# borodark/exmc

Measured on AMD Instinct MI355X. Metric: leapfrog_steps_per_s, higher is better.
Workload: dtype f64; 1 GPU; eight_schools d=10, 4096 chains/GPU (4096 total), 138450 draws/chain (2769 steps of 50 draws) after one shared 1000-iteration warmup, max_tree_depth 10, target_accept 0.8; draws_per_chain=138450, lanes_per_chain=16, warmup_lanes_per_chain=16, seed=42

## Files before the change

exmc_amd/csrc/exmc_device.hpp:

```cpp
#pragma once

#include <hip/hip_runtime.h>
#include <stdint.h>
#include <type_traits>

#include <utility>

#include "../../include/exmc_detmath.h"

namespace exmc {

constexpr uint64_t kMask58 = (1ULL << 58) - 1;

#ifndef EXMC_FIXED_PART_PIECES
#define EXMC_FIXED_PART_PIECES 7
#endif

__device__ __forceinline__ bool div_in_range(double x) {
  const uint32_t h = (uint32_t)__double2hiint(x) & 0x7fffffffu;
  return (h - 0x28300000u) < (0x57C00000u - 0x28300000u);
}

struct Recip {
  double b, r;
};

__device__ __forceinline__ Recip make_recip(double b) { return Recip{b, exmc_rcp_refined(b)}; }

__device__ __forceinline__ Recip make_recip_literal(double b) {
  __asm__ volatile("" : "+v"(b));
  return make_recip(b);
}

template <bool kFast>
struct Div {
  bool ok = true;
  __device__ __forceinline__ void watch(double x) {
    if (kFast) ok = ok && div_in_range(x);
  }
  __device__ __forceinline__ void watch_if(bool relevant, double x) {
    if (kFast) ok = ok && (!relevant || div_in_range(x));
  }
  template <int ELO, int EHI>
  __device__ __forceinline__ void watch_exp_if(bool relevant, double x) {
    static_assert(ELO >= -380 && EHI <= 380 && ELO < EHI, "inside the division window");
    if (kFast) {
      const uint32_t h = (uint32_t)__double2hiint(x) & 0x7fffffffu;
      const bool in = (h - ((uint32_t)(1023 + ELO) << 20)) < ((uint32_t)(EHI - ELO) << 20);
      ok = ok && (!relevant || in);
    }
  }
  __device__ __forceinline__ double operator()(double a, const Recip& c) const {
    return kFast ? exmc_div_core(a, c.b, c.r) : (a / c.b);
  }
  __device__ __forceinline__ double operator()(double a, double b) const {
    return kFast ? exmc_div_core(a, b, exmc_rcp_refined(b)) : (a / b);
  }
};

template <class F>
__device__ __forceinline__ double with_fast_div(F&& f) {
  Div<true> fast;
  double r = f(fast);
  if (__builtin_expect(__any(fast.ok ? 0 : 1) != 0, 0)) {
    Div<false> exact;
    r = f(exact);
  }
  return r;
// ... 1087 lines not shown
```

exmc_amd/csrc/exmc_models.hpp:

```cpp
#pragma once

#include "exmc_device.hpp"

namespace exmc {

__device__ __forceinline__ double clamp200(double z) { return fmax(-200.0, fmin(z, 200.0)); }

struct ModelDefaults {
  static constexpr bool kVregMath = false;
  static constexpr bool kCoop = false;
  static constexpr int kExtraLdsDoubles = 0;
  static constexpr int kStageDoubles = 0;
  template <class C>
  __host__ static bool stage_ok(const C&) { return true; }
  static constexpr int kStageRowOffset = 0;
  static constexpr int kLdsDataDoubles = 0;
  static constexpr bool kPipeWarmup = true;
  static constexpr bool kHasPipeWarmup = true;
  static constexpr bool kXRowLds = false;
  static constexpr bool kRowDense = false;
  static constexpr bool kLaneDense = false;
  static constexpr bool kDenseImage = false;
  static constexpr int kDenseLdsDoubles = 0;
  static constexpr int kNutsWavesPerSimd = 1;
  static constexpr bool kRngOrbit = false;
  static constexpr bool kMigrate = false;
  static constexpr double kPrioRateWith = 1.0, kPrioRateWithout = 1.0;
  static constexpr int kPipeNutsLevels = 0;
  static constexpr bool kNutsZigInLds = true;
  static constexpr bool kRegradProposal = false;
  static constexpr int kWgWaves = 0;
  static constexpr int kWgLdsLevels = 1;
  static constexpr int kWgImageDoubles = 0;
  template <class C>
  __host__ __device__ static bool wg_ok(const C&) { return false; }
  static constexpr bool kLeafPairs = false;
  static constexpr bool kLeafPairExp = false;
  static constexpr bool kLeanMomentum = false;
  static constexpr bool kPassExpPairs = false;
  static constexpr bool kOuterLogPair = false;
  static constexpr bool kTreePrefix = false;
  static constexpr bool kRngWindow = false;
  static constexpr bool kPackedTrace = false;
};

extern __shared__ double exmc_dyn_lds[];
typedef double exmc_v2d __attribute__((ext_vector_type(2)));
typedef __attribute__((address_space(3))) exmc_v2d lds_v2d;
typedef __attribute__((address_space(3))) double lds_f64_m;
static __device__ const double exmc_logtab_dev[2 * EXMC_LOGTAB_ENTRIES] = {EXMC_LOGTAB_VALUES};
__device__ static __forceinline__ double exmc_log_tab_global(double x) {
  double m;
  int e;
  const int i = exmc_logtab_split(x, &m, &e);
  return exmc_logtab_finish(m, e, exmc_logtab_dev[2 * i], exmc_logtab_dev[2 * i + 1]);
}

struct EightSchoolsConsts {
  double y[8], sg[8], lsg[8];
  double c_mu;
  double c_hc;
  double c1;
};

template <int G>
struct EightSchools : ModelDefaults {
  static constexpr int D = 10;
  static constexpr int DPL = (D + G - 1) / G;
  static constexpr bool kVregMath = (DPL <= 2);
#ifndef EXMC_ES_PIPE_LEVELS
#define EXMC_ES_PIPE_LEVELS 2
#endif
  static constexpr int kPipeNutsLevels = (G == 16) ? EXMC_ES_PIPE_LEVELS : 0;
  static constexpr bool kLeafPairs = (G == 16);
  static constexpr bool kLeafPairExp = (G == 16);
  static constexpr bool kLeanMomentum = (G == 16);
  static constexpr bool kOuterLogPair = (G == 16);
  static constexpr bool kTreePrefix = (G == 16);
  static constexpr bool kRngWindow = (G == 16);
  static constexpr bool kPackedTrace = (G == 16);
  using MM = Math<kVregMath>;
  using Consts = EightSchoolsConsts;
  struct Lane {
    double y[DPL], lsg[DPL];
    Recip sg[DPL];
    Recip five;
    double cc;
  };

  __device__ static __forceinline__ void load(const Consts& c, int l, Lane& ln) {
#pragma unroll
    for (int k = 0; k < DPL; k++) {
      const int i = l + k * G;
      const int j = (i >= 2 && i < D) ? (i - 2) : 0;
      ln.y[k] = c.y[j];
      ln.sg[k] = make_recip(c.sg[j]);
      ln.lsg[k] = c.lsg[j];
    }
    ln.five = make_recip_literal(5.0);
    ln.cc = (l == 0) ? c.c_mu : c.c1;
  }

  __device__ static __forceinline__ double logp_grad(const Consts& c, const Lane& ln, int l,
                                                     const double (&q)[DPL], double (&g)[DPL]) {
    return with_fast_div([&](auto& dv) -> double { return eval(c, ln, l, q, g, dv); });
  }

  template <class DV>
  __device__ static __forceinline__ double eval(const Consts& c, const Lane& ln, int l,
                                                const double (&q)[DPL], double (&g)[DPL], DV& dv) {
    if constexpr (kSeqSum<G, D>) return eval_row(c, ln, l, q, g, dv);
    else return eval_slots(c, ln, l, q, g, dv);
  }

  struct Mid {
    double den, zc, T, lik;
  };
  template <class DV>
  __device__ static __forceinline__ void eval_row_grad(const Consts& c, const Lane& ln, int l,
                                                       const double (&q)[DPL], double (&g)[DPL], DV& dv,
                                                       Mid& m) {
    static_assert(DPL == 1, "one dimension per lane");
    const double mu = group_bcast_c<G, 0>(q[0]);
    const double zraw = group_bcast_c<G, 1>(q[0]);
    const double zc = clamp200(zraw);
    const double tau = MM::exp_pm200(zc);
    const bool isth = (l >= 2) && (l < D);
    const bool l0 = (l == 0), l1 = (l == 1);
    const double th = q[0];
    const double theta = mu + tau * th;
    const double resid = ln.y[0] - theta;
    constexpr bool kThetaLanes = (EXMC_ROW_SUM_PIECES & 1) != 0, kOneWatch = (EXMC_ROW_SUM_PIECES & 4) != 0;
// ... 1173 lines not shown
      g[k] = (-ar) + sj * sa;
    }
    if constexpr (G == 64) rs64_allsum6(s);
    else group_allsum_n<G, 6>(s);
    const bool in_a = (zsa_raw > -200.0) && (zsa_raw < 200.0);
    const bool in_y = (zsy_raw > -200.0) && (zsy_raw < 200.0);
    if constexpr (kSpread) {
      constexpr int ks = J / G;
      const int j = l + ks * G;
      const bool is_mu = j == J, is_g = j == J + 1, is_a = j == J + 2, is_y = j == J + 3, is_b = j == J + 4;
      const double v = is_mu ? mu : (is_g ? gam : beta);
      Recip rc;
      rc.b = is_mu ? ln.ten.b : ln.five.b;
      rc.r = is_mu ? ln.ten.r : ln.five.r;
      const double cst = is_mu ? ln.kc[kMu10] : ln.kc[kN5];
      const double sx = is_mu ? s[1] : (is_g ? s[2] : s[4]);
      const double zn = dv(v - 0.0, rc);
      const double Tn = -0.5 * (zn * zn + cst);
      const double gn = (-dv(zn, rc)) + sx;
      const double zc = is_a ? za : zy, zc2 = is_a ? za2 : zy2;
      const double dc = -dv(dv(2.0 * zc, ln.c25), 1.0 + zc2);
      const double ga = in_a ? ((dc + s[3]) * sa + 1.0) : 0.0;
      const double gy = in_y ? ((dc * sy + s[5]) + 1.0) : 0.0;
      const bool is_n = is_mu || is_g || is_b;
      T[ks] = is_n ? Tn : (is_a ? t_sa : (is_y ? t_sy : T[ks]));
      g[ks] = is_n ? gn : (is_a ? ga : (is_y ? gy : g[ks]));
#pragma unroll
      for (int k = 0; k < DPL; k++)
        if (l + k * G >= D) g[k] = 0.0;
      return group_sum_slots<G, DPL>(T, valid, l, s[0]);
    }
    const double zmu = dv(mu - 0.0, ln.ten), zg = dv(gam - 0.0, ln.five), zb = dv(beta - 0.0, ln.five);
#pragma unroll
    for (int k = 0; k < DPL; k++) {
      const int j = l + k * G;
      if (j == J) { T[k] = -0.5 * (zmu * zmu + ln.kc[kMu10]); g[k] = (-dv(zmu, ln.ten)) + s[1]; }
      if (j == J + 1) { T[k] = -0.5 * (zg * zg + ln.kc[kN5]); g[k] = (-dv(zg, ln.five)) + s[2]; }
      if (j == J + 2) { T[k] = t_sa; g[k] = in_a ? ((dsa + s[3]) * sa + 1.0) : 0.0; }
      if (j == J + 3) { T[k] = t_sy; g[k] = in_y ? ((dsy * sy + s[5]) + 1.0) : 0.0; }
      if (j == J + 4) { T[k] = -0.5 * (zb * zb + ln.kc[kN5]); g[k] = (-dv(zb, ln.five)) + s[4]; }
      if (j >= D) g[k] = 0.0;
    }
    return group_sum_slots<G, DPL>(T, valid, l, s[0]);
  }
};

template <class M>
struct RowDenseModel : M {
  static constexpr bool kRowDense = true;
  static constexpr bool kPipeWarmup = false;
  static constexpr bool kOuterLogPair = false;
  static constexpr bool kTreePrefix = false;
  static constexpr bool kRngWindow = false;
  static constexpr bool kPackedTrace = false;
  static_assert(M::DPL == 1 && M::D <= 12, "row layout: one dimension per lane, D <= 12");
};

template <class M, int G>
struct LaneDenseModel : M {
  static constexpr bool kLaneDense = true;
  static constexpr bool kPipeWarmup = false;
  static constexpr int kNutsWavesPerSimd = 1;
  static constexpr int kPipeNutsLevels = 0;
  static constexpr bool kDenseImage = M::D * M::D * 8 <= 16 * 1024;
  static constexpr int kDenseLdsDoubles = (64 / G) * 3 * M::D + (kDenseImage ? M::D * M::D + 64 : 0);
  static_assert(G >= 16 && M::DPL * G >= M::D && !M::kCoop, "a lane layout that holds the whole chain");
};

}

#ifdef EXMC_CUSTOM_HEADER
#define EXMC_GEN_HOST static inline
#define EXMC_GEN_FN static __host__ __device__ __forceinline__
static __host__ __device__ __noinline__ double exmc_gen_exp_call(double x) { return exmc_exp(x); }
static __host__ __device__ __noinline__ double exmc_gen_log_call(double x) { return exmc_log(x); }
static __host__ __device__ __noinline__ double exmc_gen_log1p_call(double x) { return exmc_log1p(x); }
static __host__ __device__ __noinline__ double exmc_gen_erf_call(double x) { return exmc_erf(x); }
#define EXMC_GEN_ERF exmc_gen_erf_call
#define EXMC_GENV_ERF exmc_gen_erf_call
#ifdef EXMC_GEN_INLINE_MATH
#define EXMC_GEN_EXP exmc_exp
#define EXMC_GEN_LOG exmc_log
#define EXMC_GEN_LOG1P exmc_log1p
#else
#define EXMC_GEN_EXP exmc_gen_exp_call
#define EXMC_GEN_LOG exmc_gen_log_call
#define EXMC_GEN_LOG1P exmc_gen_log1p_call
#endif
#ifdef EXMC_GENV_CALLED_MATH
#define EXMC_GENV_EXP exmc_gen_exp_call
#define EXMC_GENV_LOG exmc_gen_log_call
#define EXMC_GENV_LOG1P exmc_gen_log1p_call
#else
#define EXMC_GENV_EXP exmc_exp
#define EXMC_GENV_LOG exmc_log
#define EXMC_GENV_LOG1P exmc_log1p
#endif
#ifdef EXMC_GENL_CALLED_MATH
#define EXMC_GENL_EXP exmc_gen_exp_call
#define EXMC_GENL_LOG exmc_gen_log_call
#define EXMC_GENL_LOG1P exmc_gen_log1p_call
#else
#define EXMC_GENL_EXP exmc::Math<true>::exp
#define EXMC_GENL_LOG exmc::Math<true>::log
#define EXMC_GENL_LOG1P exmc_log1p
#endif
// ... 409 lines not shown
```

exmc_amd/csrc/exmc_nuts.hpp:

```cpp
#pragma once

#include <type_traits>

#include "exmc_models.hpp"

#ifndef EXMC_ABLATE
#define EXMC_ABLATE 0
#endif

#ifndef EXMC_PROFILE_SECTIONS
#define EXMC_PROFILE_SECTIONS 0
#endif

namespace exmc {

#ifdef EXMC_XCC_PROBE
__device__ double g_wave_probe[4096 * 5];
#endif

#if EXMC_PROFILE_SECTIONS
__device__ unsigned long long g_prof[16];
#define EXMC_PROF_DECL long long prof_[10] = {0, 0, 0, 0, 0, 0, 0, 0, 0, 0}; long long prof_t_ = clock64();
#define EXMC_PROF(i) { const long long n_ = clock64(); prof_[i] += n_ - prof_t_; prof_t_ = n_; }
#define EXMC_PROF_COUNT(i) { prof_[i] += 1; }
// ... 1101 lines not shown
    EXMC_IPROF_COUNT
  };
  bool go_right = rng_uniform(prng) > 0.5;
  EXMC_IPROF(3)
  unit(go_right ? eps : -eps, false);
  EXMC_IPROF(1)
  for (int depth = 0;; depth++) {
    pb.sync();
    EXMC_IPROF(2)
    if (__any(pb.get_alive() ? 1 : 0) == 0) break;
    const double eps_dir = go_right ? eps : -eps;
    const int nunit = (depth == 0) ? 1 : (1 << (depth - 1));
    bool stopped = false;
    for (int i = 1; i < nunit; i++) {
      unit(eps_dir, true);
      EXMC_IPROF(1)
      pb.sync();
      EXMC_IPROF(2)
      if (__any(pb.get_alive() ? 1 : 0) == 0) { stopped = true; break; }
    }
    if (stopped) continue;
#pragma unroll
    for (int k = 0; k < DPL; k++) {
      if (go_right) { qR[k] = q[k]; pR[k] = p[k]; gR[k] = g[k]; }
      else { qL[k] = q[k]; pL[k] = p[k]; gL[k] = g[k]; }
    }
    const int nleaf = 1 << depth;
    for (int i = 0; i < nleaf; i++) rng_advance(prng);
    go_right = rng_uniform(prng) > 0.5;
#pragma unroll
    for (int k = 0; k < DPL; k++) {
      q[k] = go_right ? qR[k] : qL[k];
      p[k] = go_right ? pR[k] : pL[k];
      g[k] = go_right ? gR[k] : gL[k];
    }
    EXMC_IPROF(3)
    unit(go_right ? eps : -eps, true);
    EXMC_IPROF(1)
  }
  {
    double z[DPL];
    const Rng before = next_rng;
    draw_momentum_variates<M, G>(L, next_rng, z);
    pb.put_momentum(z, before, next_rng);
  }
  EXMC_IPROF(3)
  pb.sync();
  EXMC_IPROF(2)
  EXMC_IPROF_FLUSH
  return true;
}

template <int DPL>
struct TreeTop {
  double (&qL)[DPL], (&pL)[DPL], (&gL)[DPL], (&qR)[DPL], (&pR)[DPL], (&gR)[DPL];
  double (&rho)[DPL], (&qp)[DPL], (&gp)[DPL];
  double &logpP, &lsw, &acc;
  int &n, &depth;
  bool &div, &turn, &alive;
};

struct NoRngWindow {
  static constexpr int kOff = 0;
};
template <int I>
using IntC = std::integral_constant<int, I>;

template <class M, int G, class Win = NoRngWindow>
__device__ __forceinline__ void tree_prefix(const typename M::Consts& mc, const NutsLane<M, G>& L,
                                            double eps, double jlp0, int max_depth, Rng& trng,
                                            TreeTop<M::DPL> T, double (&q)[M::DPL], double (&p)[M::DPL],
                                            double (&g)[M::DPL], Win* win = nullptr) {
  constexpr int DPL = M::DPL;
  using MM = Math<M::kVregMath>;
  static_assert(G >= 11, "one lane per argument of the widest batch");
  static_assert(!M::kRegradProposal, "the proposal's gradient travels with it");
  constexpr bool kWin = !std::is_same<Win, NoRngWindow>::value;
  double u[10];
  double ul = 0.0;
  if constexpr (kWin) {
    static_assert(G == 16, "a group is one DPP row");
    win->build(trng);
    ul = (double)(rng_scramble(win->own()) >> 5) * 0x1p-53;
    trng = win->template state<10>();
  } else {
#pragma unroll
    for (int i = 0; i < 10; i++) u[i] = rng_uniform(trng);
  }
  auto U = [&](auto ic) -> double {
    constexpr int I = decltype(ic)::value;
    if constexpr (kWin) return group_bcast_c<G, Win::kOff + I>(ul);
    else return u[I];
  };
  const bool r0 = U(IntC<0>{}) > 0.5, r1 = U(IntC<2>{}) > 0.5, r2 = U(IntC<5>{}) > 0.5;

  PipeLeaf<DPL> f0, f1, f2, f3, f4, f5, f6;
  auto leap = [&](double eps_dir, PipeLeaf<DPL>& lf) {
    const double h = eps_dir / 2.0;
#pragma unroll
    for (int k = 0; k < DPL; k++) p[k] = p[k] + h * g[k];
    mass_drift<M, G>(L, eps_dir, p, q);
    lf.logp = M::logp_grad(mc, L.ln, L.l, q, g);
#pragma unroll
    for (int k = 0; k < DPL; k++) p[k] = p[k] + h * g[k];
#pragma unroll
    for (int k = 0; k < DPL; k++) { lf.q[k] = q[k]; lf.p[k] = p[k]; lf.g[k] = g[k]; }
  };
  double q1[DPL], g1[DPL], q2[DPL], g2[DPL];
#pragma unroll
  for (int k = 0; k < DPL; k++) { q[k] = T.qL[k]; p[k] = T.pL[k]; g[k] = T.gL[k]; }
  leap(r0 ? eps : -eps, f0);
  const bool same01 = (r0 == r1), same12 = (r1 == r2);
#pragma unroll
  for (int k = 0; k < DPL; k++) {
    q[k] = q1[k] = same01 ? f0.q[k] : T.qL[k];
    p[k] = same01 ? f0.p[k] : T.pL[k];
    g[k] = g1[k] = same01 ? f0.g[k] : T.gL[k];
  }
  leap(r1 ? eps : -eps, f1);
  leap(r1 ? eps : -eps, f2);
#pragma unroll
  for (int k = 0; k < DPL; k++) {
    q[k] = q2[k] = same12 ? f2.q[k] : (same01 ? T.qL[k] : f0.q[k]);
    p[k] = same12 ? f2.p[k] : (same01 ? T.pL[k] : f0.p[k]);
    g[k] = g2[k] = same12 ? f2.g[k] : (same01 ? T.gL[k] : f0.g[k]);
  }
  leap(r2 ? eps : -eps, f3);
  leap(r2 ? eps : -eps, f4);
  leap(r2 ? eps : -eps, f5);
  leap(r2 ? eps : -eps, f6);

  auto scalars = [&](PipeLeaf<DPL>& lf) -> double {
    const double jlp = lf.logp - mass_ke<M, G>(L, lf.p);
    const bool fin = exmc_isfinite(jlp);
    const double dl = jlp - jlp0;
    lf.div = fin ? (dl < -1000.0) : true;
    lf.lsw = fin ? dl : -1001.0;
    return fmin(dl, 0.0);
  };
  double x[11];
  x[0] = scalars(f0); x[1] = scalars(f1); x[2] = scalars(f2); x[3] = scalars(f3);
  x[4] = scalars(f4); x[5] = scalars(f5); x[6] = scalars(f6);
  x[7] = MM::lse_arg(f1.lsw, f2.lsw);
  x[8] = MM::lse_arg(f3.lsw, f4.lsw);
  x[9] = MM::lse_arg(f5.lsw, f6.lsw);
  x[10] = MM::lse_arg(T.lsw, f0.lsw);
  lane_batch<G>(x, L.l, [](double v) { return MM::exp_le0(v); });
  auto accept = [&](PipeLeaf<DPL>& lf, double ex) { lf.acc = lf.div ? 0.0 : fmin(1.0, ex); };
  accept(f0, x[0]); accept(f1, x[1]); accept(f2, x[2]); accept(f3, x[3]);
  accept(f4, x[4]); accept(f5, x[5]); accept(f6, x[6]);

  double y[11] = {1.0 + x[7], 1.0 + x[8], 1.0 + x[9], 1.0 + x[10], 0.0, 0.0, 0.0, 0.0, 0.0, 0.0, 0.0};
  if constexpr (kWin) {
    constexpr int o = Win::kOff;
    const int l = L.l;
    const bool ge1 = (l == o) || (l == o + 2) || (l == o + 5) || (l == o + 10);
    double a = ul;
    a = (l == o) ? y[0] : a;
    a = (l == o + 2) ? y[1] : a;
    a = (l == o + 5) ? y[2] : a;
    a = (l == o + 10) ? y[3] : a;
    const double r = MM::log_main(a);
    const double v = ge1 ? exmc_log_ge1_fix(a, r) : exmc_log_unit_fix(a, r);
    y[0] = group_bcast_c<G, o>(v);
    y[1] = group_bcast_c<G, o + 2>(v);
    y[2] = group_bcast_c<G, o + 5>(v);
    y[3] = group_bcast_c<G, o + 10>(v);
    y[4] = group_bcast_c<G, o + 1>(v);
    y[5] = group_bcast_c<G, o + 3>(v);
    y[6] = group_bcast_c<G, o + 4>(v);
    y[7] = group_bcast_c<G, o + 6>(v);
    y[8] = group_bcast_c<G, o + 7>(v);
    y[9] = group_bcast_c<G, o + 8>(v);
    y[10] = group_bcast_c<G, o + 9>(v);
  } else {
    y[4] = u[1]; y[5] = u[3]; y[6] = u[4]; y[7] = u[6]; y[8] = u[7]; y[9] = u[8]; y[10] = u[9];
    double v[11];
#pragma unroll
    for (int i = 0; i < 11; i++) v[i] = y[i];
    lane_batch<G>(y, L.l, [](double a) { return MM::log_main(a); });
#pragma unroll
    for (int i = 0; i < 4; i++) y[i] = exmc_log_ge1_fix(v[i], y[i]);
#pragma unroll
    for (int i = 4; i < 11; i++) y[i] = exmc_log_unit_fix(v[i], y[i]);
  }
  const double lsw12 = MM::lse_finish(f1.lsw, f2.lsw, y[0]);
  const double lsw34 = MM::lse_finish(f3.lsw, f4.lsw, y[1]);
  const double lsw56 = MM::lse_finish(f5.lsw, f6.lsw, y[2]);
  const double c12 = f1.div ? f1.lsw : lsw12;
  const double c34 = f3.div ? f3.lsw : lsw34;
  const double c56 = f5.div ? f5.lsw : lsw56;

  auto outer = [&](const PipeUnit<DPL>& c, bool go_right, double log1pe, double logu, auto dc) {
    constexpr int depth = decltype(dc)::value;
    constexpr bool kOneTest = depth == 0 && (EXMC_ROW_SUM_PIECES & 2) != 0;
    if (!T.alive) return;
    const double lsw = MM::lse_finish(T.lsw, c.lsw, log1pe);
    const bool use_sub = logu < (c.lsw - T.lsw);
    if (use_sub) {
      T.logpP = c.logpP;
#pragma unroll
      for (int k = 0; k < DPL; k++) { T.qp[k] = c.qp[k]; T.gp[k] = c.gp[k]; }
    }
    const bool divg = T.div || c.div;
    bool turning = divg || c.turn;
    double rho[DPL];
#pragma unroll
    for (int k = 0; k < DPL; k++) rho[k] = T.rho[k] + c.rho[k];
    if (!turning) {
      double nearp[DPL], farp[DPL];
#pragma unroll
      for (int k = 0; k < DPL; k++) {
        nearp[k] = go_right ? T.pR[k] : T.pL[k];
        farp[k] = go_right ? T.pL[k] : T.pR[k];
      }
      if constexpr (kOneTest) {
        turning = mass_uturn<M, G>(L, rho, farp, c.p);
      } else {
        double s2[DPL], s3[DPL];
#pragma unroll
        for (int k = 0; k < DPL; k++) {
          s2[k] = T.rho[k] + c.pin[k];
          s3[k] = nearp[k] + c.rho[k];
        }
        bool c1, c23;
        mass_uturn3<M, G>(L, rho, farp, c.p, s2, farp, c.pin, s3, nearp, c.p, c1, c23);
        turning = c1 || c23;
      }
    }
#pragma unroll
    for (int k = 0; k < DPL; k++) {
      T.rho[k] = rho[k];
      if (go_right) { T.qR[k] = c.q[k]; T.pR[k] = c.p[k]; T.gR[k] = c.g[k]; }
      else { T.qL[k] = c.q[k]; T.pL[k] = c.p[k]; T.gL[k] = c.g[k]; }
    }
    T.lsw = lsw;
    T.n += c.n;
    T.acc = T.acc + c.acc;
    T.div = divg;
    T.turn = turning;
    T.depth = depth + 1;
    T.alive = !(T.depth >= max_depth || T.div || T.turn);
  };

  double s0q[DPL], s0g[DPL];
#pragma unroll
  for (int k = 0; k < DPL; k++) { s0q[k] = T.qL[k]; s0g[k] = T.gL[k]; }
  PipeUnit<DPL> c;
  pipe_pair_unit<M, G>(L, f0, f0, false, s0q, s0g, trng, c);
  outer(c, r0, y[3], y[4], IntC<0>{});

  double w[5] = {f2.lsw - lsw12, f4.lsw - lsw34, f6.lsw - lsw56, MM::lse_arg(lsw34, c56), MM::lse_arg(T.lsw, c12)};
  lane_batch<G>(w, L.l, [](double v) { return MM::exp_le0(v); });
  PipeUnit<DPL> c1, ca, cb;
  pipe_pair_unit<M, G>(L, f1, f2, true, q1, g1, trng, c1, [&](auto, double, double) { return lsw12; },
                       [&](auto, double, double) { return w[0]; }, [&](Rng&) { return U(IntC<3>{}); });
  pipe_pair_unit<M, G>(L, f3, f4, true, q2, g2, trng, ca, [&](auto, double, double) { return lsw34; },
                       [&](auto, double, double) { return w[1]; }, [&](Rng&) { return U(IntC<6>{}); });
  pipe_pair_unit<M, G>(L, f5, f6, true, f4.q, f4.g, trng, cb, [&](auto, double, double) { return lsw56; },
                       [&](auto, double, double) { return w[2]; }, [&](Rng&) { return U(IntC<7>{}); });
  const bool parked = !(ca.div || ca.turn);

  double z[2] = {1.0 + w[3], 1.0 + w[4]};
  {
    const double v0 = z[0], v1 = z[1];
    lane_batch<G>(z, L.l, [](double a) { return MM::log_main(a); });
    z[0] = exmc_log_ge1_fix(v0, z[0]);
    z[1] = exmc_log_ge1_fix(v1, z[1]);
  }
  const double lsw_m = MM::lse_finish(lsw34, c56, z[0]);
  outer(c1, r1, z[1], f1.div ? y[5] : y[6], IntC<1>{});

  double e[2] = {c56 - lsw_m, MM::lse_arg(T.lsw, parked ? lsw_m : c34)};
  lane_batch<G>(e, L.l, [](double v) { return MM::exp_le0(v); });
  if (parked) {
    const double um = f5.div ? U(IntC<7>{}) : U(IntC<8>{});
    const bool use_b = um < e[0];
    if (!use_b) {
      cb.logpP = ca.logpP;
#pragma unroll
      for (int k = 0; k < DPL; k++) { cb.qp[k] = ca.qp[k]; cb.gp[k] = ca.gp[k]; }
    }
    bool turning = cb.div || cb.turn;
    if (!turning) {
      double rho[DPL], s2[DPL], s3[DPL];
#pragma unroll
      for (int k = 0; k < DPL; k++) {
        rho[k] = ca.rho[k] + cb.rho[k];
        s2[k] = ca.rho[k] + cb.pin[k];
        s3[k] = ca.p[k] + cb.rho[k];
      }
      bool t1, t23;
      mass_uturn3<M, G>(L, rho, ca.pin, cb.p, s2, ca.pin, cb.pin, s3, ca.p, cb.p, t1, t23);
      turning = t1 || t23;
#pragma unroll
      for (int k = 0; k < DPL; k++) { cb.rho[k] = rho[k]; cb.pin[k] = ca.pin[k]; }
    }
    cb.lsw = lsw_m;
    cb.acc = ca.acc + cb.acc;
    cb.n = 2 + cb.n;
    cb.turn = turning;
  } else {
    cb = ca;
  }

  const double lu2 = f3.div ? y[7] : (!parked ? y[8] : (f5.div ? y[9] : y[10]));
  outer(cb, r2, MM::log_ge1(1.0 + e[1]), lu2, IntC<2>{});
}

struct NoIdle {
  __device__ __forceinline__ void operator()() const {}
};

template <class M, int G, int LDSL, class Sink, class Pipe = NoPipe, class Idle = NoIdle>
__device__ __forceinline__ void nuts_run(const typename M::Consts& mc, const NutsLane<M, G>& L,
                                         ChainRegs<M::DPL>& st, int n_draws, double eps,
                                         int max_depth, Sink&& sink, Pipe* pipe = nullptr,
                                         Idle&& idle = Idle{}) {
  constexpr int DPL = M::DPL;
  constexpr int NSLOT = nuts_nslot<M>();
  constexpr bool kRegrad = M::kRegradProposal;
  constexpr int kNodeScalars = NSLOT - 3;
  using MM = Math<M::kVregMath>;
  const int l = L.l;
  const auto& im = L.im;
  double* lstk = L.lstk;
  double* gstk = L.gstk;

  double q[DPL], p[DPL], g[DPL], qold[DPL], gold[DPL];
  double qL[DPL], pL[DPL], gL[DPL], qR[DPL], pR[DPL], gR[DPL];
  double t_rho[DPL], t_qp[DPL], t_gp[DPL];
  double c_rho[DPL], c_pin[DPL], c_qp[DPL], c_gp[DPL];
#pragma unroll
  for (int k = 0; k < DPL; k++) {
    q[k] = p[k] = g[k] = qold[k] = gold[k] = 0.0;
    qL[k] = pL[k] = gL[k] = qR[k] = pR[k] = gR[k] = 0.0;
    t_rho[k] = t_qp[k] = t_gp[k] = c_rho[k] = c_pin[k] = c_qp[k] = c_gp[k] = 0.0;
  }
  double t_logpP = 0.0, t_lsw = 0.0, t_acc = 0.0, jlp0 = 0.0;
  int t_n = 0, t_depth = 0;
  bool t_div = false, t_turn = false, go_right = true;
  double eps_dir = eps;
  Rng trng = st.rng;
  const bool has = L.alive;
  constexpr bool kPrefix = M::kTreePrefix && M::kLeafPairs && Pipe::kTreePrefix && EXMC_ABLATE == 0;
  constexpr bool kWindow = kPrefix && M::kRngWindow && G == 16 && EXMC_RNG_WINDOW_STAGE >= 1;
  constexpr bool kWinMomentum = kWindow && EXMC_RNG_WINDOW_STAGE >= 2 && DPL == 1 && M::kLeanMomentum && !M::kRowDense;
  using Win = RngRowWindow<kWinMomentum ? EXMC_RNG_WINDOW : 11>;
  Win win{0, 0};

  EXMC_PROF_DECL
  EXMC_SUBPROF_DECL
  for (int draw = 0; draw < n_draws; draw++) {
    EXMC_PROF(8)
#if EXMC_PROFILE_SECTIONS == 2
    sub_[6] += 1;
#endif
    bool alive = has;
    bool have_z = false;
    double z_pre[DPL];
#pragma unroll
    for (int k = 0; k < DPL; k++) z_pre[k] = 0.0;
    if constexpr (Pipe::kOn) {
      if (pipe->pending) {
        pipe->sync();
        pipe->pending = false;
        have_z = pipe->take_momentum(st.rng, z_pre);
      }
    }
    if (has) {
      if (have_z) {
        momentum_from_variates<M, G>(L, z_pre, pL);
      } else if (kWinMomentum && L.perm == nullptr) {
        if constexpr (kWinMomentum) {
          int left = 0;
#if EXMC_PROFILE_SECTIONS == 2
          if (draw > 0) {
            long long lw[2] = {0, 0};
            draw_momentum_window<M, G>(L, win, st.rng, z_pre, left, lw);
            EXMC_SUBPROF(0)
            sub_[0] -= lw[0];
            sub_[1] += lw[0];
            sub_[5] += lw[1];
          }
#else
          if (draw > 0) draw_momentum_window<M, G>(L, win, st.rng, z_pre, left);
#endif
          if (draw == 0 || __any((left < M::D) ? 1 : 0) != 0)
            draw_momentum_lean_from<M, G>(L, st.rng, z_pre, left, draw == 0);
          EXMC_SUBPROF(2)
          momentum_from_variates<M, G>(L, z_pre, pL);
          EXMC_SUBPROF(3)
        }
      } else {
        draw_momentum<M, G>(L, st.rng, pL);
      }
      jlp0 = st.logp - mass_ke<M, G>(L, pL);
      EXMC_SUBPROF(4)
      trng = st.rng;
#pragma unroll
      for (int k = 0; k < DPL; k++) {
        qL[k] = qR[k] = t_qp[k] = st.q[k];
        gL[k] = gR[k] = t_gp[k] = st.g[k];
        pR[k] = t_rho[k] = pL[k];
      }
      t_logpP = st.logp;
      t_lsw = 0.0;
      t_acc = 0.0;
      t_n = 0;
      t_div = t_turn = false;
      t_depth = 0;
    }
    if constexpr (Pipe::kOn) {
      pipe->put_start(st.q, pL, st.g, im, eps, jlp0, trng);
      pipe->sync();
    }
    idle();
    EXMC_PROF(0)

    if constexpr (kWindow) {
      tree_prefix<M, G, Win>(mc, L, eps, jlp0, max_depth, trng,
                             TreeTop<DPL>{qL, pL, gL, qR, pR, gR, t_rho, t_qp, t_gp, t_logpP, t_lsw, t_acc,
                                          t_n, t_depth, t_div, t_turn, alive},
                             q, p, g, &win);
      EXMC_PROF(7)
    } else if constexpr (kPrefix) {
      tree_prefix<M, G>(mc, L, eps, jlp0, max_depth, trng,
                        TreeTop<DPL>{qL, pL, gL, qR, pR, gR, t_rho, t_qp, t_gp, t_logpP, t_lsw, t_acc,
                                     t_n, t_depth, t_div, t_turn, alive},
                        q, p, g);
      EXMC_PROF(7)
    }

    for (int depth = kPrefix ? 3 : 0; Pipe::kOn || __any(alive ? 1 : 0) != 0; depth++) {
      if (alive) {
        const double u = rng_uniform(trng);
        go_right = u > 0.5;
        eps_dir = go_right ? eps : -eps;
#pragma unroll
        for (int k = 0; k < DPL; k++) {
          q[k] = go_right ? qR[k] : qL[k];
          p[k] = go_right ? pR[k] : pL[k];
          g[k] = go_right ? gR[k] : gL[k];
        }
      }
      if constexpr (Pipe::kOn) {
        pipe->put_ctrl(alive, go_right);
        pipe->sync();
        if (__any(alive ? 1 : 0) == 0) break;
      }
      EXMC_PROF(1)

      static_assert(!M::kLeafPairExp || M::kLeafPairs, "kLeafPairExp batches the exponentials of kLeafPairs' pair");
      constexpr bool kOwnPairs = M::kLeafPairs && Pipe::kLeafPairs && EXMC_ABLATE == 0;
      constexpr bool kUnits = Pipe::kOn || kOwnPairs;
      constexpr int kLvl0 = kUnits ? 1 : 0;
      const int nlev = (kUnits && depth > 0) ? depth - 1 : depth;
      const int nleaf = 1 << nlev;
      for (int leaf = 0; leaf < nleaf; leaf++) {
        if constexpr (M::kNutsWavesPerSimd == 2 && !Pipe::kOn) {
          if (L.prio_slot >= 0) {
            const int phase = (int)((clock64() >> 12) & 15);
            const bool mine = (phase < L.prio_duty) == (L.prio_slot == 0);
            if (__builtin_amdgcn_readfirstlane(mine ? 1 : 0)) __builtin_amdgcn_s_setprio(3);
            else __builtin_amdgcn_s_setprio(0);
          }
        }
        if constexpr (Pipe::kOn) {
          if (leaf > 0) pipe->sync();
        }
        if (leaf > 0 && __any(alive ? 1 : 0) == 0) break;
        EXMC_PROF_COUNT(9)
        double logp_new = 0.0, jlp = 0.0;
        PipeLeaf<DPL> la, lb;
        double lsw_ab = 0.0;
        constexpr bool kExpPairs = kOwnPairs && M::kPassExpPairs && G >= 2 && EXMC_ABLATE == 0;
        constexpr bool kLogPair = kOwnPairs && M::kOuterLogPair && G >= 2 && EXMC_ABLATE == 0;
        double e_nx = 0.0, w_b = 0.0;
        auto next_lsw = [&](int nxt) -> double {
          if (nxt >= nlev) return t_lsw;
          if (nxt < LDSL) return ((const lds_f64*)(lstk + ((size_t)nxt * NSLOT + kNodeScalars) * kNutsBlock))[0];
          return gstk[((size_t)(nxt - LDSL) * NSLOT + kNodeScalars) * kNutsBlock];
        };
        (void)next_lsw;
        if constexpr (kOwnPairs) {
          double a_nx = 0.0;
          if constexpr (kExpPairs) a_nx = next_lsw(0);
          leaf_pair<M, G>(mc, L, eps_dir, jlp0, depth > 0, q, p, g, qold, gold, la, lb, lsw_ab, a_nx, w_b, e_nx);
        } else if constexpr (!Pipe::kOn) {
          const double h = eps_dir / 2.0;
#pragma unroll
          for (int k = 0; k < DPL; k++) {
            qold[k] = q[k];
            gold[k] = g[k];
            p[k] = p[k] + h * g[k];
          }
          mass_drift<M, G>(L, eps_dir, p, q);
#if EXMC_ABLATE == 3
          logp_new = 0.0;
#pragma unroll
          for (int k = 0; k < DPL; k++) { g[k] = -q[k]; logp_new = logp_new - 0.5 * q[k] * q[k]; }
          logp_new = group_allsum<G>(logp_new);
#else
          logp_new = M::logp_grad(mc, L.ln, l, q, g);
#endif
#pragma unroll
          for (int k = 0; k < DPL; k++) p[k] = p[k] + h * g[k];
          jlp = logp_new - mass_ke<M, G>(L, p);
        }
        EXMC_PROF(2)

        if (alive) {
          bool c_div, c_turn = false;
          double c_lsw, c_acc, c_logpP;
          int c_n = 1;
          if constexpr (kUnits) {
            PipeUnit<DPL> pu;
            if constexpr (Pipe::kOn) {
              pipe->get_leaf(0, la);
              if (depth > 0) pipe->get_leaf(1, lb);
              else lb = la;
              pipe_pair_unit<M, G>(L, la, lb, depth > 0, q, g, trng, pu);
            } else {
              if constexpr (kExpPairs) {
                pipe_pair_unit<M, G>(L, la, lb, depth > 0, qold, gold, trng, pu,
                                     [&](auto, double, double) { return lsw_ab; },
                                     [&](auto, double, double) { return w_b; });
              } else {
                pipe_pair_unit<M, G>(L, la, lb, depth > 0, qold, gold, trng, pu,
                                     [&](auto, double, double) { return lsw_ab; });
              }
            }
#pragma unroll
            for (int k = 0; k < DPL; k++) {
              q[k] = pu.q[k]; p[k] = pu.p[k]; g[k] = pu.g[k];
              c_rho[k] = pu.rho[k]; c_pin[k] = pu.pin[k]; c_qp[k] = pu.qp[k]; c_gp[k] = pu.gp[k];
            }
            c_div = pu.div;
            c_turn = pu.turn;
            c_lsw = pu.lsw;
            c_acc = pu.acc;
            c_logpP = pu.logpP;
            c_n = pu.n;
          } else {
            const bool fin = exmc_isfinite(jlp);
            const double dl = jlp - jlp0;
            c_div = fin ? (dl < -1000.0) : true;
            c_lsw = fin ? dl : -1001.0;
#if EXMC_ABLATE == 4
            c_acc = fmin(1.0, 1.0 + fmin(dl, 0.0));
#else
            c_acc = fmin(1.0, MM::exp_le0(fmin(dl, 0.0)));
#endif
            c_acc = c_div ? 0.0 : c_acc;
            c_logpP = c_div ? -1.0e30 : logp_new;
#pragma unroll
            for (int k = 0; k < DPL; k++) {
              c_qp[k] = c_div ? qold[k] : q[k];
              if constexpr (!kRegrad) c_gp[k] = c_div ? gold[k] : g[k];
              c_rho[k] = p[k];
              c_pin[k] = p[k];
            }
          }
          EXMC_PROF(3)

          bool parked = false;
          const int below = 2 * leaf + 1;
          (void)below;
          for (int lvl = 0; lvl < nlev; lvl++) {
            if ((leaf >> lvl) & 1) {
              if (!parked) {
// ... 1364 lines not shown
```

Baseline: 3.852 billion leapfrog_steps/s.

## Walk NUTS subtrees in four-leaf quad units with batched transcendentals

Adds a quad-walk path for eight_schools with 16 lanes per chain. The leaf loop now integrates four leapfrog steps at a time and merges two pairs into one depth-2 unit. The exp and log calls across the four leaves are batched across lanes, and the RNG state is reconstructed from how many uniforms were drawn. The point is to halve the outer leaf-loop iterations and the number of separate transcendental batches, and so cut per-leaf scalar overhead and stack traffic. In exchange, early termination is coarser: all four leaves are computed even if the first diverges, and register pressure rises. The tree-prefix code is refactored onto the same helpers.

```diff
diff --git a/exmc_amd/csrc/exmc_device.hpp b/exmc_amd/csrc/exmc_device.hpp
--- a/exmc_amd/csrc/exmc_device.hpp
+++ b/exmc_amd/csrc/exmc_device.hpp
@@ -14,6 +14,10 @@
 
 #ifndef EXMC_FIXED_PART_PIECES
 #define EXMC_FIXED_PART_PIECES 7
+#endif
+
+#ifndef EXMC_QUAD_WALK
+#define EXMC_QUAD_WALK 1
 #endif
 
 __device__ __forceinline__ bool div_in_range(double x) {
diff --git a/exmc_amd/csrc/exmc_models.hpp b/exmc_amd/csrc/exmc_models.hpp
--- a/exmc_amd/csrc/exmc_models.hpp
+++ b/exmc_amd/csrc/exmc_models.hpp
@@ -41,6 +41,7 @@
   static constexpr bool kOuterLogPair = false;
   static constexpr bool kTreePrefix = false;
   static constexpr bool kRngWindow = false;
+  static constexpr bool kQuadWalk = false;
   static constexpr bool kPackedTrace = false;
 };
 
@@ -78,6 +79,7 @@
   static constexpr bool kOuterLogPair = (G == 16);
   static constexpr bool kTreePrefix = (G == 16);
   static constexpr bool kRngWindow = (G == 16);
+  static constexpr bool kQuadWalk = (G == 16);
   static constexpr bool kPackedTrace = (G == 16);
   using MM = Math<kVregMath>;
   using Consts = EightSchoolsConsts;
@@ -1357,6 +1359,7 @@
   static constexpr bool kOuterLogPair = false;
   static constexpr bool kTreePrefix = false;
   static constexpr bool kRngWindow = false;
+  static constexpr bool kQuadWalk = false;
   static constexpr bool kPackedTrace = false;
   static_assert(M::DPL == 1 && M::D <= 12, "row layout: one dimension per lane, D <= 12");
 };
diff --git a/exmc_amd/csrc/exmc_nuts.hpp b/exmc_amd/csrc/exmc_nuts.hpp
--- a/exmc_amd/csrc/exmc_nuts.hpp
+++ b/exmc_amd/csrc/exmc_nuts.hpp
@@ -1177,6 +1177,176 @@
 }
 
 template <int DPL>
+struct QuadLeaves {
+  PipeLeaf<DPL> &a0, &b0, &a1, &b1;
+  double (&q0)[DPL], (&g0)[DPL];
+};
+struct QuadLsw {
+  double lswA, lswB, cA, cB;
+};
+
+template <class M, int G>
+__device__ __forceinline__ void unit_leap(const typename M::Consts& mc, const NutsLane<M, G>& L, double eps_dir,
+                                          double (&q)[M::DPL], double (&p)[M::DPL], double (&g)[M::DPL],
+                                          PipeLeaf<M::DPL>& lf) {
+  constexpr int DPL = M::DPL;
+  const double h = eps_dir / 2.0;
+#pragma unroll
+  for (int k = 0; k < DPL; k++) p[k] = p[k] + h * g[k];
+  mass_drift<M, G>(L, eps_dir, p, q);
+  lf.logp = M::logp_grad(mc, L.ln, L.l, q, g);
+#pragma unroll
+  for (int k = 0; k < DPL; k++) p[k] = p[k] + h * g[k];
+#pragma unroll
+  for (int k = 0; k < DPL; k++) { lf.q[k] = q[k]; lf.p[k] = p[k]; lf.g[k] = g[k]; }
+}
+template <class M, int G>
+__device__ __forceinline__ double unit_scalars(const NutsLane<M, G>& L, double jlp0, PipeLeaf<M::DPL>& lf) {
+  const double jlp = lf.logp - mass_ke<M, G>(L, lf.p);
+  const bool fin = exmc_isfinite(jlp);
+  const double dl = jlp - jlp0;
+  lf.div = fin ? (dl < -1000.0) : true;
+  lf.lsw = fin ? dl : -1001.0;
+  return fmin(dl, 0.0);
+}
+template <int DPL>
+__device__ __forceinline__ void unit_accept(PipeLeaf<DPL>& lf, double ex) { lf.acc = lf.div ? 0.0 : fmin(1.0, ex); }
+
+template <class M, int G>
+__device__ __forceinline__ void quad_integrate(const typename M::Consts& mc, const NutsLane<M, G>& L,
+                                               double eps_dir, double (&q)[M::DPL], double (&p)[M::DPL],
+                                               double (&g)[M::DPL], const QuadLeaves<M::DPL>& Q) {
+#pragma unroll
+  for (int k = 0; k < M::DPL; k++) { Q.q0[k] = q[k]; Q.g0[k] = g[k]; }
+  unit_leap<M, G>(mc, L, eps_dir, q, p, g, Q.a0);
+  unit_leap<M, G>(mc, L, eps_dir, q, p, g, Q.b0);
+  unit_leap<M, G>(mc, L, eps_dir, q, p, g, Q.a1);
+  unit_leap<M, G>(mc, L, eps_dir, q, p, g, Q.b1);
+}
+template <class M, int G>
+__device__ __forceinline__ void quad_scalars(const NutsLane<M, G>& L, double jlp0, const QuadLeaves<M::DPL>& Q,
+                                             double (&x)[4]) {
+  x[0] = unit_scalars<M, G>(L, jlp0, Q.a0);
+  x[1] = unit_scalars<M, G>(L, jlp0, Q.b0);
+  x[2] = unit_scalars<M, G>(L, jlp0, Q.a1);
+  x[3] = unit_scalars<M, G>(L, jlp0, Q.b1);
+}
+template <class M>
+__device__ __forceinline__ void quad_lse_args(const QuadLeaves<M::DPL>& Q, double& xA, double& xB) {
+  using MM = Math<M::kVregMath>;
+  xA = MM::lse_arg(Q.a0.lsw, Q.b0.lsw);
+  xB = MM::lse_arg(Q.a1.lsw, Q.b1.lsw);
+}
+template <int DPL>
+__device__ __forceinline__ void quad_accept(const QuadLeaves<DPL>& Q, double e0, double e1, double e2, double e3) {
+  unit_accept(Q.a0, e0); unit_accept(Q.b0, e1); unit_accept(Q.a1, e2); unit_accept(Q.b1, e3);
+}
+template <class M>
+__device__ __forceinline__ void quad_lse(const QuadLeaves<M::DPL>& Q, double logA, double logB, QuadLsw& S) {
+  using MM = Math<M::kVregMath>;
+  S.lswA = MM::lse_finish(Q.a0.lsw, Q.b0.lsw, logA);
+  S.lswB = MM::lse_finish(Q.a1.lsw, Q.b1.lsw, logB);
+}
+template <int DPL>
+__device__ __forceinline__ void quad_carry(const QuadLeaves<DPL>& Q, QuadLsw& S) {
+  S.cA = Q.a0.div ? Q.a0.lsw : S.lswA;
+  S.cB = Q.a1.div ? Q.a1.lsw : S.lswB;
+}
+template <class M>
+__device__ __forceinline__ void quad_weight_args(const QuadLeaves<M::DPL>& Q, const QuadLsw& S, double& wA, double& wB,
+                                                 double& xM) {
+  using MM = Math<M::kVregMath>;
+  wA = Q.b0.lsw - S.lswA;
+  wB = Q.b1.lsw - S.lswB;
+  xM = MM::lse_arg(S.lswA, S.cB);
+}
+template <class M, int G, class UA, class UB>
+__device__ __forceinline__ bool quad_pairs(const NutsLane<M, G>& L, const QuadLeaves<M::DPL>& Q, const QuadLsw& S,
+                                           double wA, double wB, UA&& uA, UB&& uB, Rng& trng,
+                                           PipeUnit<M::DPL>& ca, PipeUnit<M::DPL>& cb) {
+  pipe_pair_unit<M, G>(L, Q.a0, Q.b0, true, Q.q0, Q.g0, trng, ca, [&](auto, double, double) { return S.lswA; },
+                       [&](auto, double, double) { return wA; }, uA);
+  pipe_pair_unit<M, G>(L, Q.a1, Q.b1, true, Q.b0.q, Q.b0.g, trng, cb, [&](auto, double, double) { return S.lswB; },
+                       [&](auto, double, double) { return wB; }, uB);
+  return !(ca.div || ca.turn);
+}
+template <class M, int G, class UM>
+__device__ __forceinline__ void quad_merge(const NutsLane<M, G>& L, const PipeUnit<M::DPL>& ca, PipeUnit<M::DPL>& cb,
+                                           bool parked, UM&& um, double e_m, double lsw_m) {
+  constexpr int DPL = M::DPL;
+  if (parked) {
+    const bool use_b = um() < e_m;
+    if (!use_b) {
+      cb.logpP = ca.logpP;
+#pragma unroll
+      for (int k = 0; k < DPL; k++) { cb.qp[k] = ca.qp[k]; cb.gp[k] = ca.gp[k]; }
+    }
+    bool turning = cb.div || cb.turn;
+    if (!turning) {
+      double rho[DPL], s2[DPL], s3[DPL];
+#pragma unroll
+      for (int k = 0; k < DPL; k++) {
+        rho[k] = ca.rho[k] + cb.rho[k];
+        s2[k] = ca.rho[k] + cb.pin[k];
+        s3[k] = ca.p[k] + cb.rho[k];
+      }
+      bool t1, t23;
+      mass_uturn3<M, G>(L, rho, ca.pin, cb.p, s2, ca.pin, cb.pin, s3, ca.p, cb.p, t1, t23);
+      turning = t1 || t23;
+#pragma unroll
+      for (int k = 0; k < DPL; k++) { cb.rho[k] = rho[k]; cb.pin[k] = ca.pin[k]; }
+    }
+    cb.lsw = lsw_m;
+    cb.acc = ca.acc + cb.acc;
+    cb.n = 2 + cb.n;
+    cb.turn = turning;
+  } else {
+    cb = ca;
+  }
+}
+
+template <class M, int G>
+__device__ __forceinline__ void quad_unit(const typename M::Consts& mc, const NutsLane<M, G>& L, double eps_dir,
+                                          double jlp0, double (&q)[M::DPL], double (&p)[M::DPL],
+                                          double (&g)[M::DPL], const double (&u)[3], PipeUnit<M::DPL>& c,
+                                          int& drawn) {
+  constexpr int DPL = M::DPL;
+  using MM = Math<M::kVregMath>;
+  static_assert(G >= 6, "one lane per argument of the widest batch");
+  static_assert(!M::kRegradProposal, "the proposal's gradient travels with it");
+  PipeLeaf<DPL> a0, b0, a1, b1;
+  double q0[DPL], g0[DPL];
+  QuadLeaves<DPL> Q{a0, b0, a1, b1, q0, g0};
+  quad_integrate<M, G>(mc, L, eps_dir, q, p, g, Q);
+  double x[6], xs[4];
+  quad_scalars<M, G>(L, jlp0, Q, xs);
+  x[0] = xs[0]; x[1] = xs[1]; x[2] = xs[2]; x[3] = xs[3];
+  quad_lse_args<M>(Q, x[4], x[5]);
+  lane_batch<G>(x, L.l, [](double v) { return MM::exp_le0(v); });
+  quad_accept(Q, x[0], x[1], x[2], x[3]);
+  double y[2] = {1.0 + x[4], 1.0 + x[5]};
+  {
+    const double v0 = y[0], v1 = y[1];
+    lane_batch<G>(y, L.l, [](double a) { return MM::log_main(a); });
+    y[0] = exmc_log_ge1_fix(v0, y[0]);
+    y[1] = exmc_log_ge1_fix(v1, y[1]);
+  }
+  QuadLsw S;
+  quad_lse<M>(Q, y[0], y[1], S);
+  quad_carry(Q, S);
+  double w[3];
+  quad_weight_args<M>(Q, S, w[0], w[1], w[2]);
+  lane_batch<G>(w, L.l, [](double v) { return MM::exp_le0(v); });
+  Rng none{0, 0};
+  PipeUnit<DPL> ca;
+  const bool parked = quad_pairs<M, G>(L, Q, S, w[0], w[1], [&](Rng&) { return u[0]; }, [&](Rng&) { return u[1]; }, none, ca, c);
+  const double lsw_m = MM::lse_finish(S.lswA, S.cB, MM::log_ge1(1.0 + w[2]));
+  const double e_m = MM::exp_le0(S.cB - lsw_m);
+  quad_merge<M, G>(L, ca, c, parked, [&]() { return Q.a1.div ? u[1] : u[2]; }, e_m, lsw_m);
+  drawn = Q.a0.div ? 0 : (parked ? (Q.a1.div ? 2 : 3) : 1);
+}
+
+template <int DPL>
 struct TreeTop {
   double (&qL)[DPL], (&pL)[DPL], (&gL)[DPL], (&qR)[DPL], (&pR)[DPL], (&gR)[DPL];
   double (&rho)[DPL], (&qp)[DPL], (&gp)[DPL];
@@ -1220,18 +1390,9 @@
   const bool r0 = U(IntC<0>{}) > 0.5, r1 = U(IntC<2>{}) > 0.5, r2 = U(IntC<5>{}) > 0.5;
 
   PipeLeaf<DPL> f0, f1, f2, f3, f4, f5, f6;
-  auto leap = [&](double eps_dir, PipeLeaf<DPL>& lf) {
-    const double h = eps_dir / 2.0;
-#pragma unroll
-    for (int k = 0; k < DPL; k++) p[k] = p[k] + h * g[k];
-    mass_drift<M, G>(L, eps_dir, p, q);
-    lf.logp = M::logp_grad(mc, L.ln, L.l, q, g);
-#pragma unroll
-    for (int k = 0; k < DPL; k++) p[k] = p[k] + h * g[k];
-#pragma unroll
-    for (int k = 0; k < DPL; k++) { lf.q[k] = q[k]; lf.p[k] = p[k]; lf.g[k] = g[k]; }
-  };
+  auto leap = [&](double eps_dir, PipeLeaf<DPL>& lf) { unit_leap<M, G>(mc, L, eps_dir, q, p, g, lf); };
   double q1[DPL], g1[DPL], q2[DPL], g2[DPL];
+  QuadLeaves<DPL> Q{f3, f4, f5, f6, q2, g2};
 #pragma unroll
   for (int k = 0; k < DPL; k++) { q[k] = T.qL[k]; p[k] = T.pL[k]; g[k] = T.gL[k]; }
   leap(r0 ? eps : -eps, f0);
@@ -1246,34 +1407,23 @@
   leap(r1 ? eps : -eps, f2);
 #pragma unroll
   for (int k = 0; k < DPL; k++) {
-    q[k] = q2[k] = same12 ? f2.q[k] : (same01 ? T.qL[k] : f0.q[k]);
+    q[k] = same12 ? f2.q[k] : (same01 ? T.qL[k] : f0.q[k]);
     p[k] = same12 ? f2.p[k] : (same01 ? T.pL[k] : f0.p[k]);
-    g[k] = g2[k] = same12 ? f2.g[k] : (same01 ? T.gL[k] : f0.g[k]);
-  }
-  leap(r2 ? eps : -eps, f3);
-  leap(r2 ? eps : -eps, f4);
-  leap(r2 ? eps : -eps, f5);
-  leap(r2 ? eps : -eps, f6);
-
-  auto scalars = [&](PipeLeaf<DPL>& lf) -> double {
-    const double jlp = lf.logp - mass_ke<M, G>(L, lf.p);
-    const bool fin = exmc_isfinite(jlp);
-    const double dl = jlp - jlp0;
-    lf.div = fin ? (dl < -1000.0) : true;
-    lf.lsw = fin ? dl : -1001.0;
-    return fmin(dl, 0.0);
-  };
-  double x[11];
-  x[0] = scalars(f0); x[1] = scalars(f1); x[2] = scalars(f2); x[3] = scalars(f3);
-  x[4] = scalars(f4); x[5] = scalars(f5); x[6] = scalars(f6);
+    g[k] = same12 ? f2.g[k] : (same01 ? T.gL[k] : f0.g[k]);
+  }
+  quad_integrate<M, G>(mc, L, r2 ? eps : -eps, q, p, g, Q);
+
+  auto scalars = [&](PipeLeaf<DPL>& lf) -> double { return unit_scalars<M, G>(L, jlp0, lf); };
+  double x[11], xq[4];
+  x[0] = scalars(f0); x[1] = scalars(f1); x[2] = scalars(f2);
+  quad_scalars<M, G>(L, jlp0, Q, xq);
+  x[3] = xq[0]; x[4] = xq[1]; x[5] = xq[2]; x[6] = xq[3];
   x[7] = MM::lse_arg(f1.lsw, f2.lsw);
-  x[8] = MM::lse_arg(f3.lsw, f4.lsw);
-  x[9] = MM::lse_arg(f5.lsw, f6.lsw);
+  quad_lse_args<M>(Q, x[8], x[9]);
   x[10] = MM::lse_arg(T.lsw, f0.lsw);
   lane_batch<G>(x, L.l, [](double v) { return MM::exp_le0(v); });
-  auto accept = [&](PipeLeaf<DPL>& lf, double ex) { lf.acc = lf.div ? 0.0 : fmin(1.0, ex); };
-  accept(f0, x[0]); accept(f1, x[1]); accept(f2, x[2]); accept(f3, x[3]);
-  accept(f4, x[4]); accept(f5, x[5]); accept(f6, x[6]);
+  unit_accept(f0, x[0]); unit_accept(f1, x[1]); unit_accept(f2, x[2]);
+  quad_accept(Q, x[3], x[4], x[5], x[6]);
 
   double y[11] = {1.0 + x[7], 1.0 + x[8], 1.0 + x[9], 1.0 + x[10], 0.0, 0.0, 0.0, 0.0, 0.0, 0.0, 0.0};
   if constexpr (kWin) {
@@ -1310,11 +1460,10 @@
     for (int i = 4; i < 11; i++) y[i] = exmc_log_unit_fix(v[i], y[i]);
   }
   const double lsw12 = MM::lse_finish(f1.lsw, f2.lsw, y[0]);
-  const double lsw34 = MM::lse_finish(f3.lsw, f4.lsw, y[1]);
-  const double lsw56 = MM::lse_finish(f5.lsw, f6.lsw, y[2]);
+  QuadLsw S;
+  quad_lse<M>(Q, y[1], y[2], S);
   const double c12 = f1.div ? f1.lsw : lsw12;
-  const double c34 = f3.div ? f3.lsw : lsw34;
-  const double c56 = f5.div ? f5.lsw : lsw56;
+  quad_carry(Q, S);
 
   auto outer = [&](const PipeUnit<DPL>& c, bool go_right, double log1pe, double logu, auto dc) {
     constexpr int depth = decltype(dc)::value;
@@ -1375,16 +1524,16 @@
   pipe_pair_unit<M, G>(L, f0, f0, false, s0q, s0g, trng, c);
   outer(c, r0, y[3], y[4], IntC<0>{});
 
-  double w[5] = {f2.lsw - lsw12, f4.lsw - lsw34, f6.lsw - lsw56, MM::lse_arg(lsw34, c56), MM::lse_arg(T.lsw, c12)};
+  double w[5];
+  w[0] = f2.lsw - lsw12;
+  quad_weight_args<M>(Q, S, w[1], w[2], w[3]);
+  w[4] = MM::lse_arg(T.lsw, c12);
   lane_batch<G>(w, L.l, [](double v) { return MM::exp_le0(v); });
   PipeUnit<DPL> c1, ca, cb;
   pipe_pair_unit<M, G>(L, f1, f2, true, q1, g1, trng, c1, [&](auto, double, double) { return lsw12; },
                        [&](auto, double, double) { return w[0]; }, [&](Rng&) { return U(IntC<3>{}); });
-  pipe_pair_unit<M, G>(L, f3, f4, true, q2, g2, trng, ca, [&](auto, double, double) { return lsw34; },
-                       [&](auto, double, double) { return w[1]; }, [&](Rng&) { return U(IntC<6>{}); });
-  pipe_pair_unit<M, G>(L, f5, f6, true, f4.q, f4.g, trng, cb, [&](auto, double, double) { return lsw56; },
-                       [&](auto, double, double) { return w[2]; }, [&](Rng&) { return U(IntC<7>{}); });
-  const bool parked = !(ca.div || ca.turn);
+  const bool parked = quad_pairs<M, G>(L, Q, S, w[1], w[2], [&](Rng&) { return U(IntC<6>{}); },
+                                       [&](Rng&) { return U(IntC<7>{}); }, trng, ca, cb);
 
   double z[2] = {1.0 + w[3], 1.0 + w[4]};
   {
@@ -1393,43 +1542,14 @@
     z[0] = exmc_log_ge1_fix(v0, z[0]);
     z[1] = exmc_log_ge1_fix(v1, z[1]);
   }
-  const double lsw_m = MM::lse_finish(lsw34, c56, z[0]);
+  const double lsw_m = MM::lse_finish(S.lswA, S.cB, z[0]);
   outer(c1, r1, z[1], f1.div ? y[5] : y[6], IntC<1>{});
 
-  double e[2] = {c56 - lsw_m, MM::lse_arg(T.lsw, parked ? lsw_m : c34)};
+  double e[2] = {S.cB - lsw_m, MM::lse_arg(T.lsw, parked ? lsw_m : S.cA)};
   lane_batch<G>(e, L.l, [](double v) { return MM::exp_le0(v); });
-  if (parked) {
-    const double um = f5.div ? U(IntC<7>{}) : U(IntC<8>{});
-    const bool use_b = um < e[0];
-    if (!use_b) {
-      cb.logpP = ca.logpP;
-#pragma unroll
-      for (int k = 0; k < DPL; k++) { cb.qp[k] = ca.qp[k]; cb.gp[k] = ca.gp[k]; }
-    }
-    bool turning = cb.div || cb.turn;
-    if (!turning) {
-      double rho[DPL], s2[DPL], s3[DPL];
-#pragma unroll
-      for (int k = 0; k < DPL; k++) {
-        rho[k] = ca.rho[k] + cb.rho[k];
-        s2[k] = ca.rho[k] + cb.pin[k];
-        s3[k] = ca.p[k] + cb.rho[k];
-      }
-      bool t1, t23;
-      mass_uturn3<M, G>(L, rho, ca.pin, cb.p, s2, ca.pin, cb.pin, s3, ca.p, cb.p, t1, t23);
-      turning = t1 || t23;
-#pragma unroll
-      for (int k = 0; k < DPL; k++) { cb.rho[k] = rho[k]; cb.pin[k] = ca.pin[k]; }
-    }
-    cb.lsw = lsw_m;
-    cb.acc = ca.acc + cb.acc;
-    cb.n = 2 + cb.n;
-    cb.turn = turning;
-  } else {
-    cb = ca;
-  }
-
-  const double lu2 = f3.div ? y[7] : (!parked ? y[8] : (f5.div ? y[9] : y[10]));
+  quad_merge<M, G>(L, ca, cb, parked, [&]() { return Q.a1.div ? U(IntC<7>{}) : U(IntC<8>{}); }, e[0], lsw_m);
+
+  const double lu2 = Q.a0.div ? y[7] : (!parked ? y[8] : (Q.a1.div ? y[9] : y[10]));
   outer(cb, r2, MM::log_ge1(1.0 + e[1]), lu2, IntC<2>{});
 }
 
@@ -1473,6 +1593,8 @@
   constexpr bool kWinMomentum = kWindow && EXMC_RNG_WINDOW_STAGE >= 2 && DPL == 1 && M::kLeanMomentum && !M::kRowDense;
   using Win = RngRowWindow<kWinMomentum ? EXMC_RNG_WINDOW : 11>;
   Win win{0, 0};
+  constexpr bool kQuad = kPrefix && M::kQuadWalk && EXMC_QUAD_WALK != 0;
+  static_assert(!kQuad || !M::kPassExpPairs, "the quad pass carries no exponential ahead");
 
   EXMC_PROF_DECL
   EXMC_SUBPROF_DECL
@@ -1579,8 +1701,8 @@
       static_assert(!M::kLeafPairExp || M::kLeafPairs, "kLeafPairExp batches the exponentials of kLeafPairs' pair");
       constexpr bool kOwnPairs = M::kLeafPairs && Pipe::kLeafPairs && EXMC_ABLATE == 0;
       constexpr bool kUnits = Pipe::kOn || kOwnPairs;
-      constexpr int kLvl0 = kUnits ? 1 : 0;
-      const int nlev = (kUnits && depth > 0) ? depth - 1 : depth;
+      constexpr int kLvl0 = kQuad ? 2 : (kUnits ? 1 : 0);
+      const int nlev = kQuad ? depth - 2 : ((kUnits && depth > 0) ? depth - 1 : depth);
       const int nleaf = 1 << nlev;
       for (int leaf = 0; leaf < nleaf; leaf++) {
         if constexpr (M::kNutsWavesPerSimd == 2 && !Pipe::kOn) {
@@ -1608,7 +1730,21 @@
           return gstk[((size_t)(nxt - LDSL) * NSLOT + kNodeScalars) * kNutsBlock];
         };
         (void)next_lsw;
-        if constexpr (kOwnPairs) {
+        PipeUnit<DPL> qu;
+        int qu_drawn = 0;
+        Rng qrng[4];
+        (void)qu_drawn;
+        if constexpr (kQuad) {
+          double uq[3];
+          qrng[0] = trng;
+          Rng r = trng;
+#pragma unroll
+          for (int i = 0; i < 3; i++) {
+            uq[i] = rng_uniform(r);
+            qrng[i + 1] = r;
+          }
+          quad_unit<M, G>(mc, L, eps_dir, jlp0, q, p, g, uq, qu, qu_drawn);
+        } else if constexpr (kOwnPairs) {
           double a_nx = 0.0;
           if constexpr (kExpPairs) a_nx = next_lsw(0);
           leaf_pair<M, G>(mc, L, eps_dir, jlp0, depth > 0, q, p, g, qold, gold, la, lb, lsw_ab, a_nx, w_b, e_nx);
@@ -1641,7 +1777,13 @@
           int c_n = 1;
           if constexpr (kUnits) {
             PipeUnit<DPL> pu;
-            if constexpr (Pipe::kOn) {
+            if constexpr (kQuad) {
+              pu = qu;
+              trng = qrng[1];
+              if (qu_drawn == 0) trng = qrng[0];
+              if (qu_drawn == 2) trng = qrng[2];
+              if (qu_drawn == 3) trng = qrng[3];
+            } else if constexpr (Pipe::kOn) {
               pipe->get_leaf(0, la);
               if (depth > 0) pipe->get_leaf(1, lb);
               else lb = la;
```

After: 3.859 billion leapfrog_steps/s, median of 6. No clear change (+0.2%).
